# yirongjie/mllm

Measured on AMD Instinct MI355X. Metric: decode tok/s + prefill ms (448px img), Qwen2-VL-2B INT4, 1 GPU, higher is better.
Workload: dtype int8xint4->int32, fp32 accumulate (Q8_K x Q4_K); 1 GPU; demo_qwen2_vl Qwen2-VL-2B Q4_K: 448x448 image (1024 patches) + 24-token prompt prefill (S=282), then greedy decode, KV limit 800; parallelism=single, rccl_world=1, kv_segments=5

## Files before the change

mllm_amd/csrc/common.h:

```cpp
#pragma once
#include <hip/hip_runtime.h>
#include <hip/hip_fp16.h>
#include <stdint.h>

#include "../../include/mllm_hip.h"

namespace mllm_hip {

void set_error(const char *what, hipError_t e, const char *file, int line);
void set_error_msg(const char *fmt, ...);
int check_launch(const char *what, const char *file, int line);

#define MH_CHECK(expr)                                                        \
    do {                                                                      \
        hipError_t _e = (expr);                                               \
        if (_e != hipSuccess) {                                               \
            ::mllm_hip::set_error(#expr, _e, __FILE__, __LINE__);             \
            return MLLM_HIP_ERR_HIP;                                          \
        }                                                                     \
    } while (0)
#define MH_LAUNCH_OK(name) ::mllm_hip::check_launch(name, __FILE__, __LINE__)

static inline hipStream_t as_stream(void *s) { return reinterpret_cast<hipStream_t>(s); }

// ... 139 lines not shown
}
__device__ __forceinline__ float wave_scan_max(float v) {
    v = fmaxf(v, MH_DPPF(v, v, 0x111 , 0xF));
    v = fmaxf(v, MH_DPPF(v, v, 0x112 , 0xF));
    v = fmaxf(v, MH_DPPF(v, v, 0x114 , 0xF));
    v = fmaxf(v, MH_DPPF(v, v, 0x118 , 0xF));
    v = fmaxf(v, MH_DPPF(v, v, DPP_BCAST15, 0xA));
    v = fmaxf(v, MH_DPPF(v, v, DPP_BCAST31, 0xC));
    return v;
}
__device__ __forceinline__ float wave_shift_up(float v, float first) { return MH_DPPF(first, v, 0x138 , 0xF); }

__device__ __forceinline__ void unpack_q4k_scales(uint32_t u0, uint32_t u1, uint32_t u2, uint32_t sc8[2], uint32_t mn8[2]) {
    const uint32_t kmask1 = 0x3f3f3f3f, kmask2 = 0x0f0f0f0f, kmask3 = 0x03030303;
    mn8[1] = ((u2 >> 4) & kmask2) | (((u1 >> 6) & kmask3) << 4);
    mn8[0] = u1 & kmask1;
    sc8[1] = (u2 & kmask2) | (((u0 >> 6) & kmask3) << 4);
    sc8[0] = u0 & kmask1;
}
__device__ __forceinline__ int byte_of(const uint32_t v[2], int j) { return (v[j >> 2] >> (8 * (j & 3))) & 0xff; }

__device__ __forceinline__ int dot4(int a, int b, int c) { return __builtin_amdgcn_sdot4(a, b, c, false); }

constexpr size_t Q4KP_W_PER_BLK = 32 * 512, Q4KP_M_PER_BLK = 32 * 4 * 8, Q4KP_D_PER_BLK = 32 * 8;
__host__ __device__ static inline size_t q4kp_tile_blocks(int rows, int nb) { return (size_t)((rows + 31) / 32) * nb; }
static inline size_t q4kp_bytes(int rows, int K) {
    const size_t tb = q4kp_tile_blocks(rows, K / 256);
    return tb * (Q4KP_W_PER_BLK + Q4KP_M_PER_BLK + Q4KP_D_PER_BLK);
}
constexpr size_t Q4KW_Q_PER_BLK = 4096, Q4KW_S_PER_BLK = 512, Q4KW_M_PER_BLK = 1024, Q4KW_D_PER_BLK = 256;
static inline size_t q4kw_bytes(int rows, int K) { return q4kp_tile_blocks(rows, K / 256) * (Q4KW_Q_PER_BLK + Q4KW_S_PER_BLK + Q4KW_M_PER_BLK + Q4KW_D_PER_BLK); }

}

#include "ref_arith.h"
```

mllm_amd/csrc/kernels_elem.hip:

```cpp
#include <algorithm>
#include <vector>
#include <cmath>
#include <cstring>

#include "common.h"
#include "decode_launch.h"

namespace mllm_hip {

__device__ __forceinline__ void wave_quant_q8k(float4 v, int lane, int8_t *qs_blk, float *d_out, int16_t *bsums_blk) {
    unsigned abits;
    const float mx = q8k_first_max(v, abits);
    const float iscale = abits ? __fdiv_rn(-128.0f, mx) : 0.0f, dd = abits ? __fdiv_rn(1.0f, iscale) : 0.0f;
    uint32_t b[4];
    q8k_round4(v, iscale, b);
    const uint32_t packed = q8k_bytes(b);
    reinterpret_cast<uint32_t *>(qs_blk)[lane] = packed;
    const int s = group4_sum(q8k_sum4(packed));
    if ((lane & 3) == 0) bsums_blk[lane >> 2] = (int16_t)s;
    if (lane == 0) *d_out = dd;
}

typedef _Float16 v4h_t __attribute__((ext_vector_type(4)));
#ifndef QP_WAVES
#define QP_WAVES 8
#endif
__device__ __forceinline__ void wave_quant_pack(float4 v, int lane, bool live, uint8_t *pack, size_t tb, int nb, int m, int i) {
    unsigned abits;
    const float mx = q8k_first_max(v, abits);
    const bool nz = live && abits != 0;
    const float iscale = nz ? __fdiv_rn(-128.0f, mx) : 0.0f, dd = nz ? __fdiv_rn(1.0f, iscale) : 0.0f;
    uint32_t b[4];
    q8k_round4(v, iscale, b);
    f32x2_t q01, q23;
    q8k_floats(b, q01, q23);
    const size_t tile = (size_t)(m >> 5) * nb + i;
    const int mi = m & 31, j = lane >> 4, hf = (lane >> 3) & 1, t = lane & 7;
    v4h_t o;
    o[0] = (_Float16)q01.x; o[1] = (_Float16)q01.y; o[2] = (_Float16)q23.x; o[3] = (_Float16)q23.y;
    *reinterpret_cast<v4h_t *>(pack + ((((tile * 8 + t) * 2 + (j >> 1)) * 64 + (j & 1) * 32 + mi) * 16) + hf * 8) = o;
    const int s8 = group8_sum(q8k_sum4(q8k_bytes(b)));
    const int s8n = MH_DPP(0, s8, 0x108 , 0xF);
    if ((lane & 15) == 0) {
        v4h_t mo;
        mo[0] = (_Float16)(float)(s8 & ~1); mo[1] = (_Float16)(float)(s8 & 1);
        mo[2] = (_Float16)(float)(s8n & ~1); mo[3] = (_Float16)(float)(s8n & 1);
        *reinterpret_cast<v4h_t *>(pack + tb * Q4KP_W_PER_BLK + ((tile * 4 + (lane >> 4)) * 32 + mi) * 8) = mo;
    }
    if (lane == 0) *reinterpret_cast<float *>(pack + tb * (Q4KP_W_PER_BLK + Q4KP_M_PER_BLK) + (tile * 32 + mi) * 4) = dd;
}
__global__ __launch_bounds__(64 * QP_WAVES) void quantize_q8k_pack_kernel(const float *__restrict__ x, uint8_t *__restrict__ pack, int M, int nb) {
    const int lane = threadIdx.x & 63;
    const int64_t blk = (int64_t)blockIdx.x * QP_WAVES + (threadIdx.x >> 6);
    const int Mp = (M + 31) & ~31;
    if (blk >= (int64_t)Mp * nb) return;
    const int mi = (int)(blk & 31), i = (int)((blk >> 5) % nb), m = (int)((blk >> 5) / nb) * 32 + mi;
    const bool live = m < M;
    float4 v = make_float4(0, 0, 0, 0);
    if (live) v = reinterpret_cast<const float4 *>(x + ((int64_t)m * nb + i) * 256)[lane];
    wave_quant_pack(v, lane, live, pack, q4kp_tile_blocks(M, nb), nb, m, i);
}
__global__ __launch_bounds__(256) void quantize_q8k_kernel(const float *__restrict__ x, int8_t *__restrict__ qs, float *__restrict__ d,
                                                           int16_t *__restrict__ bsums, int64_t n_blocks) {
    const int lane = threadIdx.x & 63;
    const int64_t blk = (int64_t)blockIdx.x * 4 + (threadIdx.x >> 6);
    if (blk >= n_blocks) return;
    const float4 v = reinterpret_cast<const float4 *>(x + blk * 256)[lane];
    wave_quant_q8k(v, lane, qs + blk * 256, d + blk, bsums + blk * 16);
}

__global__ __launch_bounds__(256) void quantize_q80_kernel(const float *__restrict__ x, int8_t *__restrict__ qs, uint16_t *__restrict__ d, int64_t n_blocks) {
// ... 1292 lines not shown
```

mllm_amd/csrc/kernels_linear.hip:

```cpp
#include <type_traits>
#include <atomic>

#include "common.h"
#include "q4k_dot.h"
#include "q40_dot.h"

namespace mllm_hip {

typedef int v4i __attribute__((ext_vector_type(4)));
typedef int v16i __attribute__((ext_vector_type(16)));
typedef float v16f __attribute__((ext_vector_type(16)));

template <int NSTEPS, int ROWS>
__global__ __launch_bounds__(256) void gemv_q4k_kernel(const uint8_t *__restrict__ W, const float *__restrict__ bias, const int8_t *__restrict__ xqs,
                                                       const float *__restrict__ xd, const int16_t *__restrict__ xbsums, void *__restrict__ y, int y_f16,
                                                       const float *__restrict__ residual, int N, int nb, int rows_per_wave, int M, int64_t ldy) {
    __shared__ float2 tab_all[4 * (ROWS < 4 ? ROWS : 4) * NSTEPS * 8 * Q4K_SLOTS];
    const int lane = threadIdx.x & 63, g = lane >> 3, wid = threadIdx.x >> 6;
    const int wave = blockIdx.x * 4 + wid;
    float2 *tab = tab_all + wid * (ROWS < 4 ? ROWS : 4) * NSTEPS * 8 * Q4K_SLOTS;
    Q4KAct<NSTEPS> A;
    if (M == 1) q4k_load_act_planes<NSTEPS>(A, xqs, xd, xbsums, nb, lane);
    const int qoff = q4k_lane_qoff(lane);
    const int row0 = wave * rows_per_wave;
// ... 135 lines not shown
    float *Ad = reinterpret_cast<float *>(out + tb * (Q4KP_W_PER_BLK + Q4KP_M_PER_BLK));
    const size_t tile = (size_t)(m >> 5) * nb + i;
    const int min_ = m & 31, p = j >> 1, h = j & 1;
    const bool live = m < M;
    const int8_t *xb = xqs + ((int64_t)(live ? m : 0) * nb + i) * 256 + 64 * j;
    const uint4 la = *reinterpret_cast<const uint4 *>(xb), lb = *reinterpret_cast<const uint4 *>(xb + 16);
    const uint4 ha = *reinterpret_cast<const uint4 *>(xb + 32), hb = *reinterpret_cast<const uint4 *>(xb + 48);
    const uint32_t lo[8] = {la.x, la.y, la.z, la.w, lb.x, lb.y, lb.z, lb.w}, hi[8] = {ha.x, ha.y, ha.z, ha.w, hb.x, hb.y, hb.z, hb.w};
#pragma unroll
    for (int t = 0; t < 8; ++t) {
        v8h o;
#pragma unroll
        for (int bb = 0; bb < 4; ++bb) {
            o[bb] = (_Float16)(live ? (float)(int8_t)((lo[t] >> (8 * bb)) & 0xff) : 0.0f);
            o[4 + bb] = (_Float16)(live ? (float)(int8_t)((hi[t] >> (8 * bb)) & 0xff) : 0.0f);
        }
        Ax[((tile * 8 + t) * 2 + p) * 64 + h * 32 + min_] = o;
    }
    const int16_t *bs = xbsums + ((int64_t)(live ? m : 0) * nb + i) * 16 + 4 * j;
    const int q0 = live ? (int)bs[0] + (int)bs[1] : 0, q1 = live ? (int)bs[2] + (int)bs[3] : 0;
    v4h mo;
    mo[0] = (_Float16)(float)(q0 & ~1); mo[1] = (_Float16)(float)(q0 & 1);
    mo[2] = (_Float16)(float)(q1 & ~1); mo[3] = (_Float16)(float)(q1 & 1);
    Am[(tile * 4 + j) * 32 + min_] = mo;
    if (j == 0) Ad[tile * 32 + min_] = live ? xd[(int64_t)m * nb + i] : 0.0f;
}

constexpr int GQ_SLOT = 16384, GQ_SLOTS = 4, GQ_LDS = GQ_SLOT * GQ_SLOTS;
typedef _Float16 v2h __attribute__((ext_vector_type(2)));
__device__ __forceinline__ uint32_t and_or(uint32_t q, uint32_t mask_s, uint32_t magic_v) {
    uint32_t r;
    asm("v_and_or_b32 %0, %1, %2, %3" : "=v"(r) : "v"(q), "s"(mask_s), "v"(magic_v));
    return r;
}
__device__ __forceinline__ v8h q4_expand(uint32_t q, v2h s, v2h o1024, v2h o64, uint32_t m0f, uint32_t mf0, uint32_t k1024, uint32_t k64) {
    const uint32_t t = q >> 8;
    const v2h d0 = __builtin_bit_cast(v2h, and_or(q, m0f, k1024)), d1 = __builtin_bit_cast(v2h, and_or(q, mf0, k64));
    const v2h d2 = __builtin_bit_cast(v2h, and_or(t, m0f, k1024)), d3 = __builtin_bit_cast(v2h, and_or(t, mf0, k64));
    const v2h w0 = __builtin_elementwise_fma(d0, (v2h){s[0], s[0]}, (v2h){o1024[0], o1024[0]});
    const v2h w1 = __builtin_elementwise_fma(d1, (v2h){s[0], s[0]}, (v2h){o64[0], o64[0]});
    const v2h w2 = __builtin_elementwise_fma(d2, (v2h){s[1], s[1]}, (v2h){o1024[1], o1024[1]});
    const v2h w3 = __builtin_elementwise_fma(d3, (v2h){s[1], s[1]}, (v2h){o64[1], o64[1]});
    return (v8h){w0[0], w0[1], w1[0], w1[1], w2[0], w2[1], w3[0], w3[1]};
}
#if defined(MLLM_HIP_STAMPS)
constexpr int GQ_ST_HS = 12, GQ_ST_N = 8, GQ_ST_WG = 64;
__device__ unsigned long long g_gq_stamps[GQ_ST_WG * (4 * GQ_ST_HS * GQ_ST_N + 8)];
#define GQS(i) do { __builtin_amdgcn_sched_barrier(0); const unsigned long long t_ = __builtin_amdgcn_s_memtime(); if (lane == 0 && st_hs < GQ_ST_HS) st_lds[(wid * GQ_ST_HS + st_hs) * GQ_ST_N + (i)] = t_; __builtin_amdgcn_sched_barrier(0); } while (0)
#else
#define GQS(i) do { } while (0)
#endif
#if defined(GQ_NO_RETIRE)
constexpr int GQ_RET = 1;
#else
constexpr int GQ_RET = 16;
#endif
#if defined(GQ_NO_MFMA)
#define GQ_MFMA(a, b, c) (c)
#else
#define GQ_MFMA(a, b, c) __builtin_amdgcn_mfma_f32_32x32x16_f16(a, b, c, 0, 0, 0)
#endif
#if defined(GQ_NO_EXPAND)
#define GQ_EXPAND(q, s, o1, o2) __builtin_bit_cast(v8h, (u32x4){q, q, q, q})
#else
#define GQ_EXPAND(q, s, o1, o2) q4_expand(q, s, o1, o2, m0f, mf0, k1024, k64)
#endif
__global__ __launch_bounds__(256, 2) void gemm_q4k_kernel(const uint8_t *__restrict__ Wp, const uint8_t *__restrict__ Xp, const float *__restrict__ bias,
                                                          void *__restrict__ y, int y_f16, int64_t ldy, const float *__restrict__ residual, int M, int N,
                                                          int nb, int m_fastest) {
    extern __shared__ __attribute__((aligned(16))) char ring[];
    const int GXt = (N + 63) / 64, MTt = (M + 31) / 32;
    const int tile_x = m_fastest ? (int)blockIdx.x / MTt : (int)blockIdx.x % GXt, tile_y = m_fastest ? (int)blockIdx.x % MTt : (int)blockIdx.x / GXt;
    const int lane = threadIdx.x & 63, wid = __builtin_amdgcn_readfirstlane(threadIdx.x >> 6);
#if defined(MLLM_HIP_STAMPS)
    __shared__ unsigned long long st_lds[4 * GQ_ST_HS * GQ_ST_N];
    int st_hs = 0;
    unsigned long long st_rt[6];
    st_rt[0] = __builtin_amdgcn_s_memrealtime();
    st_rt[2] = 0;
    for (int i = threadIdx.x; i < 4 * GQ_ST_HS * GQ_ST_N; i += 256) st_lds[i] = 0;
#endif
#if defined(GQ_STAGGER)
    if ((((int)blockIdx.x >> 8) & 1) && (int)blockIdx.x < 512) {
#pragma unroll 1
        for (int i = 0; i < GQ_STAGGER; i += 100) __builtin_amdgcn_s_sleep(100);
    }
#endif
    const int col = lane & 31, h = lane >> 5;
    const int NT = (N + 31) / 32;
    const int nw = wid >> 1, ch = wid & 1;
    const int mt = tile_y, nt = tile_x * 2 + nw;
    const bool active = nt < NT;
    const size_t tbw = q4kp_tile_blocks(N, nb), tbx = q4kp_tile_blocks(M, nb);
    const int nts0 = min(tile_x * 2, NT - 1), nts1 = min(tile_x * 2 + 1, NT - 1);
    const uint8_t *XpM = Xp + tbx * Q4KP_W_PER_BLK, *XpD = XpM + tbx * Q4KP_M_PER_BLK;
    const uint8_t *WpS = Wp + tbw * Q4KW_Q_PER_BLK, *WpM = WpS + tbw * Q4KW_S_PER_BLK, *WpD = WpM + tbw * Q4KW_M_PER_BLK;
    const unsigned ring0 = (unsigned)(size_t)ring;
    auto uniform_ptr = [](const uint8_t *ptr) __attribute__((always_inline)) {
        const uint32_t plo = (uint32_t)__builtin_amdgcn_readfirstlane((int)(uint32_t)(uint64_t)ptr), phi = (uint32_t)__builtin_amdgcn_readfirstlane((int)(uint32_t)((uint64_t)ptr >> 32));
        return reinterpret_cast<const uint8_t *>(((uint64_t)phi << 32) | (uint64_t)plo);
    };
    const uint8_t *sa0 = uniform_ptr(Xp + (size_t)mt * nb * Q4KP_W_PER_BLK + (size_t)wid * 1024);
    const uint8_t *sa1 = uniform_ptr(Xp + (size_t)mt * nb * Q4KP_W_PER_BLK + (size_t)(4 + wid) * 1024);
    const uint8_t *sq = uniform_ptr(Wp + (size_t)(nw ? nts1 : nts0) * nb * Q4KW_Q_PER_BLK + (size_t)ch * 1024);
    const uint8_t *pe = Xp + lane * 16, *po = Xp + lane * 16;
    unsigned se = 0, so = 0;
    if (wid == 0) {
        pe = lane < 8    ? XpD + (size_t)mt * nb * 128 + lane * 16
             : lane < 24 ? WpD + (size_t)nts0 * nb * 256 + (lane - 8) * 16
             : lane < 40 ? WpD + (size_t)nts1 * nb * 256 + (lane - 24) * 16
                         : Xp + lane * 16;
        se = lane < 8 ? 128u : (lane < 40 ? 256u : 0u);
        po = XpM + (size_t)mt * nb * 1024 + lane * 16;
        so = 1024u;
    } else if (wid == 1) {
        pe = WpS + (size_t)(lane < 32 ? nts0 : nts1) * nb * 512 + (lane & 31) * 16;
        se = 512u;
        po = WpM + (size_t)nts0 * nb * 1024 + lane * 16;
        so = 1024u;
    } else if (wid == 2) {
        po = WpM + (size_t)nts1 * nb * 1024 + lane * 16;
        so = 1024u;
    }
    unsigned voffA = (unsigned)lane * 16u, voffB = (unsigned)lane * 16u;
    unsigned islot = ring0;
    auto issue = [&](int hb) __attribute__((always_inline)) {
        const unsigned d0 = __builtin_amdgcn_readfirstlane(islot + (unsigned)wid * 1024u);
        const uint8_t *pa = hb == 0 ? pe : po;
        unsigned keep;
        asm volatile("s_mov_b32 %0, m0\n\ts_mov_b32 m0, %3\n\ts_nop 0\n\tglobal_load_lds_dwordx4 %1, %4\n\t"
                     "s_add_u32 m0, m0, 0x1000\n\ts_nop 0\n\tglobal_load_lds_dwordx4 %1, %5\n\t"
                     "s_add_u32 m0, m0, 0x1000\n\ts_nop 0\n\tglobal_load_lds_dwordx4 %2, %6\n\t"
                     "s_add_u32 m0, m0, 0x1000\n\ts_nop 0\n\tglobal_load_lds_dwordx4 %7, off\n\ts_mov_b32 m0, %0"
                     : "=&s"(keep) : "v"(voffA), "v"(voffB), "s"(d0), "s"(sa0), "s"(sa1), "s"(sq), "v"(pa) : "memory", "scc");
        voffA += 8192u;
        voffB += 2048u;
        islot = islot + (unsigned)GQ_SLOT == ring0 + (unsigned)GQ_LDS ? ring0 : islot + (unsigned)GQ_SLOT;
        if (hb == 0) pe += se; else po += so;
    };
    const int TS = 2 * nb;
    issue(0);
    issue(1);
    if (TS > 2) issue(0);
    __builtin_amdgcn_sched_barrier(0);
#if defined(MLLM_HIP_STAMPS)
    st_rt[1] = __builtin_amdgcn_s_memrealtime();
#endif
    v16f acc[4], accm[2];
#pragma unroll
    for (int t = 0; t < 4; ++t)
#pragma unroll
        for (int r = 0; r < 16; ++r) acc[t][r] = 0.0f;
#pragma unroll
    for (int u = 0; u < 2; ++u)
#pragma unroll
        for (int r = 0; r < 16; ++r) accm[u][r] = 0.0f;
    v16f zero;
#pragma unroll
    for (int r = 0; r < 16; ++r) zero[r] = 0.0f;
    typedef float f32x4 __attribute__((ext_vector_type(4)));
    typedef float f32x2 __attribute__((ext_vector_type(2)));
    typedef unsigned u32x2 __attribute__((ext_vector_type(2)));
    typedef unsigned u32x4 __attribute__((ext_vector_type(4)));
    float dd[16], dm[16];
#pragma unroll
    for (int r = 0; r < 16; ++r) dd[r] = dm[r] = 0.0f;
    v16f cp0 = zero, cp1 = zero;
    v2h sc[2] = {{0, 0}, {0, 0}}, o1024[2] = {{0, 0}, {0, 0}}, o64[2] = {{0, 0}, {0, 0}};
    const uint32_t k1024 = 0x64006400u, k64 = 0x54005400u;
    const uint32_t m0f = __builtin_amdgcn_readfirstlane(0x000F000F), mf0 = __builtin_amdgcn_readfirstlane(0x00F000F0);
    const unsigned lA = ring0 + (unsigned)(ch * 4096 + lane * 16), lQ = ring0 + (unsigned)((8 + 2 * nw + ch) * 1024 + lane * 16);
    const unsigned lX = ring0 + (unsigned)(12288 + 16 * h), lW = ring0 + (unsigned)(12288 + 128 + nw * 256 + col * 8), lS = ring0 + (unsigned)(13312 + nw * 512 + lane * 8);
    const unsigned lAm = ring0 + (unsigned)(12288 + col * 8 + 2 * ch * 256), lBm = ring0 + (unsigned)(13312 + nw * 1024 + col * 8 + 2 * ch * 256);
    unsigned cslot = 0;
    auto step = [&](auto HB, auto REM) __attribute__((always_inline)) {
        constexpr int hb = decltype(HB)::value, rem = decltype(REM)::value;
        GQS(0);
        if (rem >= 2) asm volatile("s_waitcnt vmcnt(8)" ::: "memory");
        else if (rem == 1) asm volatile("s_waitcnt vmcnt(4)" ::: "memory");
        else asm volatile("s_waitcnt vmcnt(0)" ::: "memory");
        GQS(1);
#if !defined(GQ_NO_BAR)
        __builtin_amdgcn_s_barrier();
#endif
        asm volatile("" ::: "memory");
        GQS(2);
#if defined(MLLM_HIP_STAMPS)
        if (st_rt[2] == 0) st_rt[2] = __builtin_amdgcn_s_memrealtime();
#endif
#if !defined(GQ_NO_DMA)
        if (rem >= 3) issue(1 - hb);
#endif
        GQS(3);
        if (active) {
            typedef __attribute__((address_space(3))) const char *lds_cp;
            const unsigned cs = __builtin_amdgcn_readfirstlane(cslot);
            const u32x4 qv = *reinterpret_cast<__attribute__((address_space(3))) const u32x4 *>((lds_cp)(size_t)(lQ + cs));
            u32x2 sraw;
            if (hb == 0) sraw = *reinterpret_cast<__attribute__((address_space(3))) const u32x2 *>((lds_cp)(size_t)(lS + cs));
            const __attribute__((address_space(3))) v8h *A = reinterpret_cast<__attribute__((address_space(3))) const v8h *>((lds_cp)(size_t)(lA + cs));
            const v8h a0 = A[0], a2 = A[128], a1 = A[64], a3 = A[192];
            f32x2 dwv;
            f32x4 dx[4];
            v4h a4[2], b4[2];
            if (hb == 0) {
                dwv = *reinterpret_cast<__attribute__((address_space(3))) const f32x2 *>((lds_cp)(size_t)(lW + cs));
#pragma unroll
                for (int g4 = 0; g4 < 4; ++g4) dx[g4] = *reinterpret_cast<__attribute__((address_space(3))) const f32x4 *>((lds_cp)(size_t)(lX + cs) + 32 * g4);
            } else {
                const __attribute__((address_space(3))) v4h *Am = reinterpret_cast<__attribute__((address_space(3))) const v4h *>((lds_cp)(size_t)(lAm + cs));
                const __attribute__((address_space(3))) v4h *Bm = reinterpret_cast<__attribute__((address_space(3))) const v4h *>((lds_cp)(size_t)(lBm + cs));
#pragma unroll
                for (int k = 0; k < 2; ++k) { a4[k] = Am[k * 32]; b4[k] = Bm[k * 32]; }
            }
            GQS(4);
#pragma unroll
            for (int r = 0; r < GQ_RET; ++r) acc[2 * (1 - hb)][r] = __fmaf_rn(dd[r], cp0[r], acc[2 * (1 - hb)][r]);
            if (hb == 0) {
                const v2h n1024 = {(_Float16)-1024.0f, (_Float16)-1024.0f}, n64 = {(_Float16)-64.0f, (_Float16)-64.0f};
#pragma unroll
                for (int p = 0; p < 2; ++p) {
                    const unsigned sv = p == 0 ? sraw.x : sraw.y;
                    sc[p] = __builtin_bit_cast(v2h, sv);
                    o1024[p] = sc[p] * n1024;
                    o64[p] = sc[p] * n64;
                }
            }
            v16f cm0, cm1;
            if (hb == 1) {
                v8h am[2], bm[2];
#pragma unroll
                for (int k = 0; k < 2; ++k) {
                    const u32x2 ua = __builtin_bit_cast(u32x2, a4[k]), ub = __builtin_bit_cast(u32x2, b4[k]);
                    const u32x4 wa = {h == 0 ? ua[0] : 0u, h == 0 ? ua[1] : 0u, 0u, 0u}, wb = {h == 0 ? ub[0] : 0u, h == 0 ? ub[1] : 0u, 0u, 0u};
                    am[k] = __builtin_bit_cast(v8h, wa); bm[k] = __builtin_bit_cast(v8h, wb);
                }
                cm0 = GQ_MFMA(am[0], bm[0], zero);
                cm1 = GQ_MFMA(am[1], bm[1], zero);
            }
            const v8h b0 = GQ_EXPAND(qv[0], sc[0], o1024[0], o64[0]);
            cp0 = GQ_MFMA(a0, b0, zero);
#pragma unroll
            for (int r = 0; r < GQ_RET; ++r) acc[2 * (1 - hb) + 1][r] = __fmaf_rn(dd[r], cp1[r], acc[2 * (1 - hb) + 1][r]);
            const v8h b2 = GQ_EXPAND(qv[2], sc[0], o1024[0], o64[0]);
            cp1 = GQ_MFMA(a2, b2, zero);
            const v8h b1 = GQ_EXPAND(qv[1], sc[1], o1024[1], o64[1]);
            cp0 = GQ_MFMA(a1, b1, cp0);
            const v8h b3 = GQ_EXPAND(qv[3], sc[1], o1024[1], o64[1]);
            cp1 = GQ_MFMA(a3, b3, cp1);
            if (hb == 0) {
#pragma unroll
                for (int g4 = 0; g4 < 4; ++g4)
#pragma unroll
                    for (int e = 0; e < 4; ++e) {
                        dd[4 * g4 + e] = dx[g4][e] * dwv[0];
                        dm[4 * g4 + e] = (-dx[g4][e]) * dwv[1];
                    }
            } else {
#pragma unroll
                for (int r = 0; r < 16; ++r) {
                    accm[0][r] = __fmaf_rn(dm[r], cm0[r], accm[0][r]);
                    accm[1][r] = __fmaf_rn(dm[r], cm1[r], accm[1][r]);
                }
            }
        }
        GQS(6);
#if defined(MLLM_HIP_STAMPS)
        ++st_hs;
#endif
        cslot = cslot + (unsigned)GQ_SLOT == (unsigned)GQ_LDS ? 0u : cslot + (unsigned)GQ_SLOT;
    };
    using std::integral_constant;
#pragma unroll 1
    for (int i = 0; i + 2 < nb; ++i) {
        step(integral_constant<int, 0>{}, integral_constant<int, 3>{});
        step(integral_constant<int, 1>{}, integral_constant<int, 3>{});
    }
    if (nb >= 2) {
        step(integral_constant<int, 0>{}, integral_constant<int, 3>{});
        step(integral_constant<int, 1>{}, integral_constant<int, 2>{});
    }
    step(integral_constant<int, 0>{}, integral_constant<int, 1>{});
    step(integral_constant<int, 1>{}, integral_constant<int, 0>{});
    if (active) {
#pragma unroll
        for (int r = 0; r < 16; ++r) {
            acc[2][r] = __fmaf_rn(dd[r], cp0[r], acc[2][r]);
            acc[3][r] = __fmaf_rn(dd[r], cp1[r], acc[3][r]);
        }
    }
#if defined(MLLM_HIP_STAMPS)
    st_rt[3] = __builtin_amdgcn_s_memrealtime();
#endif
    float x[16], yv[16];
#pragma unroll
    for (int r = 0; r < 16; ++r) { x[r] = acc[0][r] + acc[2][r]; yv[r] = acc[1][r] + acc[3][r]; }
    __syncthreads();
    float *xch = reinterpret_cast<float *>(ring) + (size_t)nw * 64 * 64 + lane;
    const int n = nt * 32 + col;
    auto finish = [&](auto R0) __attribute__((always_inline)) {
        constexpr int r0 = decltype(R0)::value, p0 = 8 - r0;
#pragma unroll
        for (int j = 0; j < 8; ++j) {
            const int r = p0 + j;
            xch[r * 64] = x[r]; xch[(16 + r) * 64] = yv[r]; xch[(32 + r) * 64] = accm[0][r]; xch[(48 + r) * 64] = accm[1][r];
        }
        __syncthreads();
#if defined(MLLM_HIP_STAMPS)
        st_rt[4] = __builtin_amdgcn_s_memrealtime();
#endif
        if (!active || n >= N) return;
        float v[8];
#pragma unroll
        for (int j = 0; j < 8; ++j) {
            const int r = r0 + j;
            const float hs = (x[r] + xch[r * 64]) + (yv[r] + xch[(16 + r) * 64]);
            v[j] = hs + ((accm[0][r] + xch[(32 + r) * 64]) + (accm[1][r] + xch[(48 + r) * 64]));
        }
        if (bias) {
            const float bv = bias[n];
#pragma unroll
            for (int j = 0; j < 8; ++j) v[j] = v[j] + bv;
        }
        const int mb = mt * 32 + 4 * h;
        if (y_f16) {
            uint16_t *yp = reinterpret_cast<uint16_t *>(y) + n;
#pragma unroll
            for (int j = 0; j < 8; ++j) {
                const int m = mb + ((r0 + j) & 3) + 8 * ((r0 + j) >> 2);
                if (m < M) yp[(int64_t)m * ldy] = f2h(v[j]);
            }
        } else {
            float *yp = reinterpret_cast<float *>(y) + n;
            if (residual) {
                float res[8];
#pragma unroll
                for (int j = 0; j < 8; ++j) res[j] = residual[(int64_t)min(mb + ((r0 + j) & 3) + 8 * ((r0 + j) >> 2), M - 1) * ldy + n];
#pragma unroll
                for (int j = 0; j < 8; ++j) v[j] = v[j] + res[j];
            }
#pragma unroll
            for (int j = 0; j < 8; ++j) {
                const int m = mb + ((r0 + j) & 3) + 8 * ((r0 + j) >> 2);
                if (m < M) yp[(int64_t)m * ldy] = v[j];
            }
        }
    };
    if (ch == 0) finish(std::integral_constant<int, 0>{}); else finish(std::integral_constant<int, 8>{});
#if defined(MLLM_HIP_STAMPS)
    {
        const int wg = blockIdx.x;
        if (wg % 37 == 0 && wg / 37 < GQ_ST_WG) {
            unsigned long long *dst = g_gq_stamps + (size_t)(wg / 37) * (4 * GQ_ST_HS * GQ_ST_N + 8);
            for (int i = threadIdx.x; i < 4 * GQ_ST_HS * GQ_ST_N; i += 256) dst[i] = st_lds[i];
            asm volatile("s_waitcnt vmcnt(0)" ::: "memory");
            st_rt[5] = __builtin_amdgcn_s_memrealtime();
            if (threadIdx.x == 0) {
                unsigned long long *tail = dst + 4 * GQ_ST_HS * GQ_ST_N;
                for (int i = 0; i < 6; ++i) tail[i] = st_rt[i];
                tail[6] = __builtin_amdgcn_s_getreg(63492); tail[7] = __builtin_amdgcn_s_getreg(63508);
            }
        }
    }
#endif
}

#if defined(MLLM_HIP_STAMPS)
extern "C" int mllm_hip_debug_read_gemm_stamps(unsigned long long *host, int n) {
    return hipMemcpyFromSymbol(host, HIP_SYMBOL(g_gq_stamps), (size_t)n * 8) == hipSuccess ? 0 : -1;
}
#endif

constexpr int F32_TM = 8, F32_TN = 4;
#define SWZ_XOR(v, k) __int_as_float(__builtin_amdgcn_ds_swizzle(__float_as_int(v), 0x1f | ((k) << 10)))
__global__ __launch_bounds__(256) void gemm_f32_kernel(const float *__restrict__ W, const float *__restrict__ bias, const float *__restrict__ x,
                                                       float *__restrict__ y, int64_t ldy, int M, int N, int K) {
    const int c = threadIdx.x & 31, gi = threadIdx.x >> 5;
    const int m0 = blockIdx.y * (2 * F32_TM) + (gi >> 2) * F32_TM, n0 = blockIdx.x * (4 * F32_TN) + (gi & 3) * F32_TN;
    const float *xr[F32_TM], *wr[F32_TN];
#pragma unroll
    for (int i = 0; i < F32_TM; ++i) xr[i] = x + (int64_t)min(m0 + i, M - 1) * K;
#pragma unroll
    for (int j = 0; j < F32_TN; ++j) wr[j] = W + (int64_t)min(n0 + j, N - 1) * K;
    float acc[F32_TM][F32_TN];
#pragma unroll
    for (int i = 0; i < F32_TM; ++i)
#pragma unroll
        for (int j = 0; j < F32_TN; ++j) acc[i][j] = 0.0f;
    const int np = K & ~31;
    for (int k = c; k < np; k += 32) {
        float xv[F32_TM], wv[F32_TN];
#pragma unroll
        for (int i = 0; i < F32_TM; ++i) xv[i] = xr[i][k];
#pragma unroll
// ... 391 lines not shown
```

Measured before the change: 1206 tok/s.

## Restructure Q4_K GEMM LDS ring layout and DMA addressing to cut loop bookkeeping

Reworks the prefill Q4_K MFMA GEMM's LDS staging. The per-step ring-slot modulo arithmetic is replaced by ping-pong base pointers that flip each super-block. DMA issues now use immediate offsets instead of m0 increments, and the activation min-sum plane is widened to 64 entries (zero-padded), so wave 3 also gets a DMA stream. Debug stamp and ablation macros are removed and a script is added to count loop instructions. The aim is fewer scalar and vector bookkeeping instructions per super-block, at the cost of a larger packed activation buffer and extra zero writes.

Measured after the change: 1205 tok/s. No clear change (-0.0%).

```diff
diff --git a/mllm_amd/csrc/common.h b/mllm_amd/csrc/common.h
--- a/mllm_amd/csrc/common.h
+++ b/mllm_amd/csrc/common.h
@@ -185,7 +185,7 @@
 
 __device__ __forceinline__ int dot4(int a, int b, int c) { return __builtin_amdgcn_sdot4(a, b, c, false); }
 
-constexpr size_t Q4KP_W_PER_BLK = 32 * 512, Q4KP_M_PER_BLK = 32 * 4 * 8, Q4KP_D_PER_BLK = 32 * 8;
+constexpr size_t Q4KP_W_PER_BLK = 32 * 512, Q4KP_M_PER_BLK = 64 * 4 * 8, Q4KP_D_PER_BLK = 32 * 8;
 __host__ __device__ static inline size_t q4kp_tile_blocks(int rows, int nb) { return (size_t)((rows + 31) / 32) * nb; }
 static inline size_t q4kp_bytes(int rows, int K) {
     const size_t tb = q4kp_tile_blocks(rows, K / 256);
diff --git a/mllm_amd/csrc/kernels_elem.hip b/mllm_amd/csrc/kernels_elem.hip
--- a/mllm_amd/csrc/kernels_elem.hip
+++ b/mllm_amd/csrc/kernels_elem.hip
@@ -45,8 +45,10 @@
         v4h_t mo;
         mo[0] = (_Float16)(float)(s8 & ~1); mo[1] = (_Float16)(float)(s8 & 1);
         mo[2] = (_Float16)(float)(s8n & ~1); mo[3] = (_Float16)(float)(s8n & 1);
-        *reinterpret_cast<v4h_t *>(pack + tb * Q4KP_W_PER_BLK + ((tile * 4 + (lane >> 4)) * 32 + mi) * 8) = mo;
-    }
+        *reinterpret_cast<v4h_t *>(pack + tb * Q4KP_W_PER_BLK + ((tile * 4 + (lane >> 4)) * 64 + mi) * 8) = mo;
+    }
+    if ((lane & 15) == 8)
+        *reinterpret_cast<v4h_t *>(pack + tb * Q4KP_W_PER_BLK + ((tile * 4 + (lane >> 4)) * 64 + 32 + mi) * 8) = (v4h_t){(_Float16)0.0f, (_Float16)0.0f, (_Float16)0.0f, (_Float16)0.0f};
     if (lane == 0) *reinterpret_cast<float *>(pack + tb * (Q4KP_W_PER_BLK + Q4KP_M_PER_BLK) + (tile * 32 + mi) * 4) = dd;
 }
 __global__ __launch_bounds__(64 * QP_WAVES) void quantize_q8k_pack_kernel(const float *__restrict__ x, uint8_t *__restrict__ pack, int M, int nb) {
diff --git a/mllm_amd/csrc/kernels_linear.hip b/mllm_amd/csrc/kernels_linear.hip
--- a/mllm_amd/csrc/kernels_linear.hip
+++ b/mllm_amd/csrc/kernels_linear.hip
@@ -181,7 +181,8 @@
     v4h mo;
     mo[0] = (_Float16)(float)(q0 & ~1); mo[1] = (_Float16)(float)(q0 & 1);
     mo[2] = (_Float16)(float)(q1 & ~1); mo[3] = (_Float16)(float)(q1 & 1);
-    Am[(tile * 4 + j) * 32 + min_] = mo;
+    Am[(tile * 4 + j) * 64 + min_] = mo;
+    Am[(tile * 4 + j) * 64 + 32 + min_] = (v4h){(_Float16)0.0f, (_Float16)0.0f, (_Float16)0.0f, (_Float16)0.0f};
     if (j == 0) Ad[tile * 32 + min_] = live ? xd[(int64_t)m * nb + i] : 0.0f;
 }
 
@@ -202,28 +203,6 @@
     const v2h w3 = __builtin_elementwise_fma(d3, (v2h){s[1], s[1]}, (v2h){o64[1], o64[1]});
     return (v8h){w0[0], w0[1], w1[0], w1[1], w2[0], w2[1], w3[0], w3[1]};
 }
-#if defined(MLLM_HIP_STAMPS)
-constexpr int GQ_ST_HS = 12, GQ_ST_N = 8, GQ_ST_WG = 64;
-__device__ unsigned long long g_gq_stamps[GQ_ST_WG * (4 * GQ_ST_HS * GQ_ST_N + 8)];
-#define GQS(i) do { __builtin_amdgcn_sched_barrier(0); const unsigned long long t_ = __builtin_amdgcn_s_memtime(); if (lane == 0 && st_hs < GQ_ST_HS) st_lds[(wid * GQ_ST_HS + st_hs) * GQ_ST_N + (i)] = t_; __builtin_amdgcn_sched_barrier(0); } while (0)
-#else
-#define GQS(i) do { } while (0)
-#endif
-#if defined(GQ_NO_RETIRE)
-constexpr int GQ_RET = 1;
-#else
-constexpr int GQ_RET = 16;
-#endif
-#if defined(GQ_NO_MFMA)
-#define GQ_MFMA(a, b, c) (c)
-#else
-#define GQ_MFMA(a, b, c) __builtin_amdgcn_mfma_f32_32x32x16_f16(a, b, c, 0, 0, 0)
-#endif
-#if defined(GQ_NO_EXPAND)
-#define GQ_EXPAND(q, s, o1, o2) __builtin_bit_cast(v8h, (u32x4){q, q, q, q})
-#else
-#define GQ_EXPAND(q, s, o1, o2) q4_expand(q, s, o1, o2, m0f, mf0, k1024, k64)
-#endif
 __global__ __launch_bounds__(256, 2) void gemm_q4k_kernel(const uint8_t *__restrict__ Wp, const uint8_t *__restrict__ Xp, const float *__restrict__ bias,
                                                           void *__restrict__ y, int y_f16, int64_t ldy, const float *__restrict__ residual, int M, int N,
                                                           int nb, int m_fastest) {
@@ -231,20 +210,6 @@
     const int GXt = (N + 63) / 64, MTt = (M + 31) / 32;
     const int tile_x = m_fastest ? (int)blockIdx.x / MTt : (int)blockIdx.x % GXt, tile_y = m_fastest ? (int)blockIdx.x % MTt : (int)blockIdx.x / GXt;
     const int lane = threadIdx.x & 63, wid = __builtin_amdgcn_readfirstlane(threadIdx.x >> 6);
-#if defined(MLLM_HIP_STAMPS)
-    __shared__ unsigned long long st_lds[4 * GQ_ST_HS * GQ_ST_N];
-    int st_hs = 0;
-    unsigned long long st_rt[6];
-    st_rt[0] = __builtin_amdgcn_s_memrealtime();
-    st_rt[2] = 0;
-    for (int i = threadIdx.x; i < 4 * GQ_ST_HS * GQ_ST_N; i += 256) st_lds[i] = 0;
-#endif
-#if defined(GQ_STAGGER)
-    if ((((int)blockIdx.x >> 8) & 1) && (int)blockIdx.x < 512) {
-#pragma unroll 1
-        for (int i = 0; i < GQ_STAGGER; i += 100) __builtin_amdgcn_s_sleep(100);
-    }
-#endif
     const int col = lane & 31, h = lane >> 5;
     const int NT = (N + 31) / 32;
     const int nw = wid >> 1, ch = wid & 1;
@@ -255,56 +220,64 @@
     const uint8_t *XpM = Xp + tbx * Q4KP_W_PER_BLK, *XpD = XpM + tbx * Q4KP_M_PER_BLK;
     const uint8_t *WpS = Wp + tbw * Q4KW_Q_PER_BLK, *WpM = WpS + tbw * Q4KW_S_PER_BLK, *WpD = WpM + tbw * Q4KW_M_PER_BLK;
     const unsigned ring0 = (unsigned)(size_t)ring;
-    auto uniform_ptr = [](const uint8_t *ptr) __attribute__((always_inline)) {
-        const uint32_t plo = (uint32_t)__builtin_amdgcn_readfirstlane((int)(uint32_t)(uint64_t)ptr), phi = (uint32_t)__builtin_amdgcn_readfirstlane((int)(uint32_t)((uint64_t)ptr >> 32));
+    auto uniform_ptr = [](uintptr_t ptr) __attribute__((always_inline)) {
+        const uint32_t plo = (uint32_t)__builtin_amdgcn_readfirstlane((int)(uint32_t)ptr), phi = (uint32_t)__builtin_amdgcn_readfirstlane((int)(uint32_t)((uint64_t)ptr >> 32));
         return reinterpret_cast<const uint8_t *>(((uint64_t)phi << 32) | (uint64_t)plo);
     };
-    const uint8_t *sa0 = uniform_ptr(Xp + (size_t)mt * nb * Q4KP_W_PER_BLK + (size_t)wid * 1024);
-    const uint8_t *sa1 = uniform_ptr(Xp + (size_t)mt * nb * Q4KP_W_PER_BLK + (size_t)(4 + wid) * 1024);
-    const uint8_t *sq = uniform_ptr(Wp + (size_t)(nw ? nts1 : nts0) * nb * Q4KW_Q_PER_BLK + (size_t)ch * 1024);
-    const uint8_t *pe = Xp + lane * 16, *po = Xp + lane * 16;
+    const uint8_t *sa0 = uniform_ptr((uintptr_t)Xp + (size_t)mt * nb * Q4KP_W_PER_BLK + (size_t)wid * 1024);
+    const uint8_t *sa1 = uniform_ptr((uintptr_t)Xp + (size_t)mt * nb * Q4KP_W_PER_BLK + (size_t)(4 + wid) * 1024 - 1024);
+    const uint8_t *sq = uniform_ptr((uintptr_t)Wp + (size_t)(nw ? nts1 : nts0) * nb * Q4KW_Q_PER_BLK + (size_t)ch * 1024 - 2048);
+    uintptr_t pe = (uintptr_t)Xp + lane * 16, po = (uintptr_t)Xp + lane * 16;
     unsigned se = 0, so = 0;
     if (wid == 0) {
-        pe = lane < 8    ? XpD + (size_t)mt * nb * 128 + lane * 16
-             : lane < 24 ? WpD + (size_t)nts0 * nb * 256 + (lane - 8) * 16
-             : lane < 40 ? WpD + (size_t)nts1 * nb * 256 + (lane - 24) * 16
-                         : Xp + lane * 16;
+        pe = (uintptr_t)(lane < 8    ? XpD + (size_t)mt * nb * 128 + lane * 16
+                         : lane < 24 ? WpD + (size_t)nts0 * nb * 256 + (lane - 8) * 16
+                         : lane < 40 ? WpD + (size_t)nts1 * nb * 256 + (lane - 24) * 16
+                                     : Xp + lane * 16);
         se = lane < 8 ? 128u : (lane < 40 ? 256u : 0u);
-        po = XpM + (size_t)mt * nb * 1024 + lane * 16;
-        so = 1024u;
+        po = (uintptr_t)(XpM + (size_t)mt * nb * Q4KP_M_PER_BLK + lane * 16);
+        so = (unsigned)Q4KP_M_PER_BLK;
     } else if (wid == 1) {
-        pe = WpS + (size_t)(lane < 32 ? nts0 : nts1) * nb * 512 + (lane & 31) * 16;
+        pe = (uintptr_t)(WpS + (size_t)(lane < 32 ? nts0 : nts1) * nb * 512 + (lane & 31) * 16);
         se = 512u;
-        po = WpM + (size_t)nts0 * nb * 1024 + lane * 16;
+        po = (uintptr_t)(WpM + (size_t)nts0 * nb * 1024 + lane * 16);
         so = 1024u;
     } else if (wid == 2) {
-        po = WpM + (size_t)nts1 * nb * 1024 + lane * 16;
+        po = (uintptr_t)(WpM + (size_t)nts1 * nb * 1024 + lane * 16);
         so = 1024u;
-    }
+    } else {
+        po = (uintptr_t)(XpM + (size_t)mt * nb * Q4KP_M_PER_BLK + 1024 + lane * 16);
+        so = (unsigned)Q4KP_M_PER_BLK;
+    }
+    pe -= 3072;
+    po -= 3072;
     unsigned voffA = (unsigned)lane * 16u, voffB = (unsigned)lane * 16u;
-    unsigned islot = ring0;
-    auto issue = [&](int hb) __attribute__((always_inline)) {
-        const unsigned d0 = __builtin_amdgcn_readfirstlane(islot + (unsigned)wid * 1024u);
-        const uint8_t *pa = hb == 0 ? pe : po;
+    const unsigned dbase = __builtin_amdgcn_readfirstlane(ring0 + (unsigned)wid * 4096u);
+    auto issue = [&](auto HB, unsigned d0) __attribute__((always_inline)) {
+        constexpr int hb = decltype(HB)::value;
+        const uintptr_t pa = hb == 0 ? pe : po;
         unsigned keep;
-        asm volatile("s_mov_b32 %0, m0\n\ts_mov_b32 m0, %3\n\ts_nop 0\n\tglobal_load_lds_dwordx4 %1, %4\n\t"
-                     "s_add_u32 m0, m0, 0x1000\n\ts_nop 0\n\tglobal_load_lds_dwordx4 %1, %5\n\t"
-                     "s_add_u32 m0, m0, 0x1000\n\ts_nop 0\n\tglobal_load_lds_dwordx4 %2, %6\n\t"
-                     "s_add_u32 m0, m0, 0x1000\n\ts_nop 0\n\tglobal_load_lds_dwordx4 %7, off\n\ts_mov_b32 m0, %0"
-                     : "=&s"(keep) : "v"(voffA), "v"(voffB), "s"(d0), "s"(sa0), "s"(sa1), "s"(sq), "v"(pa) : "memory", "scc");
+        asm volatile("s_mov_b32 %0, m0\n\ts_mov_b32 m0, %3\n\ts_nop 0\n\t"
+                     "global_load_lds_dwordx4 %1, %4\n\t"
+                     "global_load_lds_dwordx4 %1, %5 offset:1024\n\t"
+                     "global_load_lds_dwordx4 %2, %6 offset:2048\n\t"
+                     "global_load_lds_dwordx4 %7, off offset:3072\n\ts_mov_b32 m0, %0"
+                     : "=&s"(keep) : "v"(voffA), "v"(voffB), "s"(d0), "s"(sa0), "s"(sa1), "s"(sq), "v"(pa) : "memory");
         voffA += 8192u;
         voffB += 2048u;
-        islot = islot + (unsigned)GQ_SLOT == ring0 + (unsigned)GQ_LDS ? ring0 : islot + (unsigned)GQ_SLOT;
         if (hb == 0) pe += se; else po += so;
     };
+    using std::integral_constant;
+    typedef integral_constant<int, 0> I0;
+    typedef integral_constant<int, 1> I1;
+    typedef integral_constant<int, 2> I2;
+    typedef integral_constant<int, 3> I3;
+    unsigned dA = dbase + 3u * GQ_SLOT, dB = dbase, sdl = 2u * GQ_SLOT;
     const int TS = 2 * nb;
-    issue(0);
-    issue(1);
-    if (TS > 2) issue(0);
+    issue(I0{}, dbase);
+    issue(I1{}, dbase + (unsigned)GQ_SLOT);
+    if (TS > 2) issue(I0{}, dbase + 2u * GQ_SLOT);
     __builtin_amdgcn_sched_barrier(0);
-#if defined(MLLM_HIP_STAMPS)
-    st_rt[1] = __builtin_amdgcn_s_memrealtime();
-#endif
     v16f acc[4], accm[2];
 #pragma unroll
     for (int t = 0; t < 4; ++t)
@@ -328,129 +301,109 @@
     v2h sc[2] = {{0, 0}, {0, 0}}, o1024[2] = {{0, 0}, {0, 0}}, o64[2] = {{0, 0}, {0, 0}};
     const uint32_t k1024 = 0x64006400u, k64 = 0x54005400u;
     const uint32_t m0f = __builtin_amdgcn_readfirstlane(0x000F000F), mf0 = __builtin_amdgcn_readfirstlane(0x00F000F0);
-    const unsigned lA = ring0 + (unsigned)(ch * 4096 + lane * 16), lQ = ring0 + (unsigned)((8 + 2 * nw + ch) * 1024 + lane * 16);
-    const unsigned lX = ring0 + (unsigned)(12288 + 16 * h), lW = ring0 + (unsigned)(12288 + 128 + nw * 256 + col * 8), lS = ring0 + (unsigned)(13312 + nw * 512 + lane * 8);
-    const unsigned lAm = ring0 + (unsigned)(12288 + col * 8 + 2 * ch * 256), lBm = ring0 + (unsigned)(13312 + nw * 1024 + col * 8 + 2 * ch * 256);
-    unsigned cslot = 0;
+    typedef __attribute__((address_space(3))) const char *lds_cp;
+    unsigned lA = ring0 + (unsigned)(ch * 1024 + lane * 16), lQ = ring0 + (unsigned)((4 * wid + 2) * 1024 + lane * 16);
+    unsigned lX = ring0 + (unsigned)(3072 + 16 * h), lW = ring0 + (unsigned)(3072 + 128 + nw * 256 + col * 8), lS = ring0 + (unsigned)(7168 + nw * 512 + lane * 8);
+    unsigned lAm = ring0 + (unsigned)((ch ? 15360 : 3072) + lane * 8), lBm = ring0 + (unsigned)(7168 + nw * 4096 + col * 8 + ch * 512);
     auto step = [&](auto HB, auto REM) __attribute__((always_inline)) {
-        constexpr int hb = decltype(HB)::value, rem = decltype(REM)::value;
-        GQS(0);
+        constexpr int hb = decltype(HB)::value, rem = decltype(REM)::value, so_ = hb * GQ_SLOT;
+        const lds_cp pA = (lds_cp)(size_t)lA, pQ = (lds_cp)(size_t)lQ, pX = (lds_cp)(size_t)lX, pW = (lds_cp)(size_t)lW, pS = (lds_cp)(size_t)lS;
+        const lds_cp pAm = (lds_cp)(size_t)lAm, pBm = (lds_cp)(size_t)lBm;
         if (rem >= 2) asm volatile("s_waitcnt vmcnt(8)" ::: "memory");
         else if (rem == 1) asm volatile("s_waitcnt vmcnt(4)" ::: "memory");
         else asm volatile("s_waitcnt vmcnt(0)" ::: "memory");
-        GQS(1);
-#if !defined(GQ_NO_BAR)
         __builtin_amdgcn_s_barrier();
-#endif
         asm volatile("" ::: "memory");
-        GQS(2);
-#if defined(MLLM_HIP_STAMPS)
-        if (st_rt[2] == 0) st_rt[2] = __builtin_amdgcn_s_memrealtime();
-#endif
-#if !defined(GQ_NO_DMA)
-        if (rem >= 3) issue(1 - hb);
-#endif
-        GQS(3);
-        if (active) {
-            typedef __attribute__((address_space(3))) const char *lds_cp;
-            const unsigned cs = __builtin_amdgcn_readfirstlane(cslot);
-            const u32x4 qv = *reinterpret_cast<__attribute__((address_space(3))) const u32x4 *>((lds_cp)(size_t)(lQ + cs));
-            u32x2 sraw;
-            if (hb == 0) sraw = *reinterpret_cast<__attribute__((address_space(3))) const u32x2 *>((lds_cp)(size_t)(lS + cs));
-            const __attribute__((address_space(3))) v8h *A = reinterpret_cast<__attribute__((address_space(3))) const v8h *>((lds_cp)(size_t)(lA + cs));
-            const v8h a0 = A[0], a2 = A[128], a1 = A[64], a3 = A[192];
-            f32x2 dwv;
-            f32x4 dx[4];
-            v4h a4[2], b4[2];
-            if (hb == 0) {
-                dwv = *reinterpret_cast<__attribute__((address_space(3))) const f32x2 *>((lds_cp)(size_t)(lW + cs));
-#pragma unroll
-                for (int g4 = 0; g4 < 4; ++g4) dx[g4] = *reinterpret_cast<__attribute__((address_space(3))) const f32x4 *>((lds_cp)(size_t)(lX + cs) + 32 * g4);
-            } else {
-                const __attribute__((address_space(3))) v4h *Am = reinterpret_cast<__attribute__((address_space(3))) const v4h *>((lds_cp)(size_t)(lAm + cs));
-                const __attribute__((address_space(3))) v4h *Bm = reinterpret_cast<__attribute__((address_space(3))) const v4h *>((lds_cp)(size_t)(lBm + cs));
-#pragma unroll
-                for (int k = 0; k < 2; ++k) { a4[k] = Am[k * 32]; b4[k] = Bm[k * 32]; }
-            }
-            GQS(4);
-#pragma unroll
-            for (int r = 0; r < GQ_RET; ++r) acc[2 * (1 - hb)][r] = __fmaf_rn(dd[r], cp0[r], acc[2 * (1 - hb)][r]);
-            if (hb == 0) {
-                const v2h n1024 = {(_Float16)-1024.0f, (_Float16)-1024.0f}, n64 = {(_Float16)-64.0f, (_Float16)-64.0f};
-#pragma unroll
-                for (int p = 0; p < 2; ++p) {
-                    const unsigned sv = p == 0 ? sraw.x : sraw.y;
-                    sc[p] = __builtin_bit_cast(v2h, sv);
-                    o1024[p] = sc[p] * n1024;
-                    o64[p] = sc[p] * n64;
+        if (rem >= 3) issue(integral_constant<int, 1 - hb>{}, hb == 0 ? dA : dB);
+        __builtin_amdgcn_sched_barrier(0);
+        const u32x4 qv = *reinterpret_cast<__attribute__((address_space(3))) const u32x4 *>(pQ + so_);
+        u32x2 sraw;
+        if (hb == 0) sraw = *reinterpret_cast<__attribute__((address_space(3))) const u32x2 *>(pS + so_);
+        const __attribute__((address_space(3))) v8h *A = reinterpret_cast<__attribute__((address_space(3))) const v8h *>(pA + so_);
+        const v8h a0 = A[0], a2 = A[512], a1 = A[256], a3 = A[768];
+        f32x2 dwv;
+        f32x4 dx[4];
+        v4h a4[2], b4[2];
+        if (hb == 0) {
+            dwv = *reinterpret_cast<__attribute__((address_space(3))) const f32x2 *>(pW + so_);
+#pragma unroll
+            for (int g4 = 0; g4 < 4; ++g4) dx[g4] = *reinterpret_cast<__attribute__((address_space(3))) const f32x4 *>(pX + so_ + 32 * g4);
+        } else {
+            const volatile __attribute__((address_space(3))) v4h *Am = reinterpret_cast<const volatile __attribute__((address_space(3))) v4h *>(pAm + so_);
+            const volatile __attribute__((address_space(3))) v4h *Bm = reinterpret_cast<const volatile __attribute__((address_space(3))) v4h *>(pBm + so_);
+#pragma unroll
+            for (int k = 0; k < 2; ++k) { a4[k] = Am[k * 64]; b4[k] = Bm[k * 32]; }
+        }
+#pragma unroll
+        for (int r = 0; r < 16; ++r) acc[2 * (1 - hb)][r] = __fmaf_rn(dd[r], cp0[r], acc[2 * (1 - hb)][r]);
+        if (hb == 0) {
+            const v2h n1024 = {(_Float16)-1024.0f, (_Float16)-1024.0f}, n64 = {(_Float16)-64.0f, (_Float16)-64.0f};
+#pragma unroll
+            for (int p = 0; p < 2; ++p) {
+                const unsigned sv = p == 0 ? sraw.x : sraw.y;
+                sc[p] = __builtin_bit_cast(v2h, sv);
+                o1024[p] = sc[p] * n1024;
+                o64[p] = sc[p] * n64;
+            }
+        }
+        v16f cm0, cm1;
+        if (hb == 1) {
+            v8h am[2], bm[2];
+#pragma unroll
+            for (int k = 0; k < 2; ++k) {
+                const u32x2 ua = __builtin_bit_cast(u32x2, a4[k]), ub = __builtin_bit_cast(u32x2, b4[k]);
+                const u32x4 wa = {ua[0], ua[1], 0u, 0u}, wb = {ub[0], ub[1], 0u, 0u};
+                am[k] = __builtin_bit_cast(v8h, wa); bm[k] = __builtin_bit_cast(v8h, wb);
+            }
+            cm0 = __builtin_amdgcn_mfma_f32_32x32x16_f16(am[0], bm[0], zero, 0, 0, 0);
+            cm1 = __builtin_amdgcn_mfma_f32_32x32x16_f16(am[1], bm[1], zero, 0, 0, 0);
+        }
+        const v8h b0 = q4_expand(qv[0], sc[0], o1024[0], o64[0], m0f, mf0, k1024, k64);
+        cp0 = __builtin_amdgcn_mfma_f32_32x32x16_f16(a0, b0, zero, 0, 0, 0);
+#pragma unroll
+        for (int r = 0; r < 16; ++r) acc[2 * (1 - hb) + 1][r] = __fmaf_rn(dd[r], cp1[r], acc[2 * (1 - hb) + 1][r]);
+        const v8h b2 = q4_expand(qv[2], sc[0], o1024[0], o64[0], m0f, mf0, k1024, k64);
+        cp1 = __builtin_amdgcn_mfma_f32_32x32x16_f16(a2, b2, zero, 0, 0, 0);
+        const v8h b1 = q4_expand(qv[1], sc[1], o1024[1], o64[1], m0f, mf0, k1024, k64);
+        cp0 = __builtin_amdgcn_mfma_f32_32x32x16_f16(a1, b1, cp0, 0, 0, 0);
+        const v8h b3 = q4_expand(qv[3], sc[1], o1024[1], o64[1], m0f, mf0, k1024, k64);
+        cp1 = __builtin_amdgcn_mfma_f32_32x32x16_f16(a3, b3, cp1, 0, 0, 0);
+        if (hb == 0) {
+#pragma unroll
+            for (int g4 = 0; g4 < 4; ++g4)
+#pragma unroll
+                for (int e = 0; e < 4; ++e) {
+                    dd[4 * g4 + e] = dx[g4][e] * dwv[0];
+                    dm[4 * g4 + e] = (-dx[g4][e]) * dwv[1];
                 }
-            }
-            v16f cm0, cm1;
-            if (hb == 1) {
-                v8h am[2], bm[2];
-#pragma unroll
-                for (int k = 0; k < 2; ++k) {
-                    const u32x2 ua = __builtin_bit_cast(u32x2, a4[k]), ub = __builtin_bit_cast(u32x2, b4[k]);
-                    const u32x4 wa = {h == 0 ? ua[0] : 0u, h == 0 ? ua[1] : 0u, 0u, 0u}, wb = {h == 0 ? ub[0] : 0u, h == 0 ? ub[1] : 0u, 0u, 0u};
-                    am[k] = __builtin_bit_cast(v8h, wa); bm[k] = __builtin_bit_cast(v8h, wb);
-                }
-                cm0 = GQ_MFMA(am[0], bm[0], zero);
-                cm1 = GQ_MFMA(am[1], bm[1], zero);
-            }
-            const v8h b0 = GQ_EXPAND(qv[0], sc[0], o1024[0], o64[0]);
-            cp0 = GQ_MFMA(a0, b0, zero);
-#pragma unroll
-            for (int r = 0; r < GQ_RET; ++r) acc[2 * (1 - hb) + 1][r] = __fmaf_rn(dd[r], cp1[r], acc[2 * (1 - hb) + 1][r]);
-            const v8h b2 = GQ_EXPAND(qv[2], sc[0], o1024[0], o64[0]);
-            cp1 = GQ_MFMA(a2, b2, zero);
-            const v8h b1 = GQ_EXPAND(qv[1], sc[1], o1024[1], o64[1]);
-            cp0 = GQ_MFMA(a1, b1, cp0);
-            const v8h b3 = GQ_EXPAND(qv[3], sc[1], o1024[1], o64[1]);
-            cp1 = GQ_MFMA(a3, b3, cp1);
-            if (hb == 0) {
-#pragma unroll
-                for (int g4 = 0; g4 < 4; ++g4)
-#pragma unroll
-                    for (int e = 0; e < 4; ++e) {
-                        dd[4 * g4 + e] = dx[g4][e] * dwv[0];
-                        dm[4 * g4 + e] = (-dx[g4][e]) * dwv[1];
-                    }
-            } else {
-#pragma unroll
-                for (int r = 0; r < 16; ++r) {
-                    accm[0][r] = __fmaf_rn(dm[r], cm0[r], accm[0][r]);
-                    accm[1][r] = __fmaf_rn(dm[r], cm1[r], accm[1][r]);
-                }
-            }
-        }
-        GQS(6);
-#if defined(MLLM_HIP_STAMPS)
-        ++st_hs;
-#endif
-        cslot = cslot + (unsigned)GQ_SLOT == (unsigned)GQ_LDS ? 0u : cslot + (unsigned)GQ_SLOT;
+        } else {
+#pragma unroll
+            for (int r = 0; r < 16; ++r) {
+                accm[0][r] = __fmaf_rn(dm[r], cm0[r], accm[0][r]);
+                accm[1][r] = __fmaf_rn(dm[r], cm1[r], accm[1][r]);
+            }
+            if (rem > 0) {
+                lA += sdl; lQ += sdl; lX += sdl; lW += sdl; lS += sdl; lAm += sdl; lBm += sdl;
+                dA -= sdl; dB += sdl; sdl = 0u - sdl;
+            }
+        }
     };
-    using std::integral_constant;
 #pragma unroll 1
     for (int i = 0; i + 2 < nb; ++i) {
-        step(integral_constant<int, 0>{}, integral_constant<int, 3>{});
-        step(integral_constant<int, 1>{}, integral_constant<int, 3>{});
+        step(I0{}, I3{});
+        step(I1{}, I3{});
     }
     if (nb >= 2) {
-        step(integral_constant<int, 0>{}, integral_constant<int, 3>{});
-        step(integral_constant<int, 1>{}, integral_constant<int, 2>{});
-    }
-    step(integral_constant<int, 0>{}, integral_constant<int, 1>{});
-    step(integral_constant<int, 1>{}, integral_constant<int, 0>{});
-    if (active) {
-#pragma unroll
-        for (int r = 0; r < 16; ++r) {
-            acc[2][r] = __fmaf_rn(dd[r], cp0[r], acc[2][r]);
-            acc[3][r] = __fmaf_rn(dd[r], cp1[r], acc[3][r]);
-        }
-    }
-#if defined(MLLM_HIP_STAMPS)
-    st_rt[3] = __builtin_amdgcn_s_memrealtime();
-#endif
+        step(I0{}, I3{});
+        step(I1{}, I2{});
+    }
+    step(I0{}, I1{});
+    step(I1{}, I0{});
+#pragma unroll
+    for (int r = 0; r < 16; ++r) {
+        acc[2][r] = __fmaf_rn(dd[r], cp0[r], acc[2][r]);
+        acc[3][r] = __fmaf_rn(dd[r], cp1[r], acc[3][r]);
+    }
     float x[16], yv[16];
 #pragma unroll
     for (int r = 0; r < 16; ++r) { x[r] = acc[0][r] + acc[2][r]; yv[r] = acc[1][r] + acc[3][r]; }
@@ -465,9 +418,6 @@
             xch[r * 64] = x[r]; xch[(16 + r) * 64] = yv[r]; xch[(32 + r) * 64] = accm[0][r]; xch[(48 + r) * 64] = accm[1][r];
         }
         __syncthreads();
-#if defined(MLLM_HIP_STAMPS)
-        st_rt[4] = __builtin_amdgcn_s_memrealtime();
-#endif
         if (!active || n >= N) return;
         float v[8];
 #pragma unroll
@@ -506,29 +456,7 @@
         }
     };
     if (ch == 0) finish(std::integral_constant<int, 0>{}); else finish(std::integral_constant<int, 8>{});
-#if defined(MLLM_HIP_STAMPS)
-    {
-        const int wg = blockIdx.x;
-        if (wg % 37 == 0 && wg / 37 < GQ_ST_WG) {
-            unsigned long long *dst = g_gq_stamps + (size_t)(wg / 37) * (4 * GQ_ST_HS * GQ_ST_N + 8);
-            for (int i = threadIdx.x; i < 4 * GQ_ST_HS * GQ_ST_N; i += 256) dst[i] = st_lds[i];
-            asm volatile("s_waitcnt vmcnt(0)" ::: "memory");
-            st_rt[5] = __builtin_amdgcn_s_memrealtime();
-            if (threadIdx.x == 0) {
-                unsigned long long *tail = dst + 4 * GQ_ST_HS * GQ_ST_N;
-                for (int i = 0; i < 6; ++i) tail[i] = st_rt[i];
-                tail[6] = __builtin_amdgcn_s_getreg(63492); tail[7] = __builtin_amdgcn_s_getreg(63508);
-            }
-        }
-    }
-#endif
-}
-
-#if defined(MLLM_HIP_STAMPS)
-extern "C" int mllm_hip_debug_read_gemm_stamps(unsigned long long *host, int n) {
-    return hipMemcpyFromSymbol(host, HIP_SYMBOL(g_gq_stamps), (size_t)n * 8) == hipSuccess ? 0 : -1;
-}
-#endif
+}
 
 constexpr int F32_TM = 8, F32_TN = 4;
 #define SWZ_XOR(v, k) __int_as_float(__builtin_amdgcn_ds_swizzle(__float_as_int(v), 0x1f | ((k) << 10)))
diff --git a/profiles/gemm_loop_count.py b/profiles/gemm_loop_count.py
--- /dev/null
+++ b/profiles/gemm_loop_count.py
@@ -0,0 +1,76 @@
+#!/usr/bin/env python3
+import collections
+import os
+import re
+import subprocess
+import sys
+import tempfile
+
+HERE = os.path.dirname(os.path.abspath(__file__))
+ARITH = ("v_and_or_b32", "v_pk_fma_f16", "v_lshrrev_b32", "v_pk_mul_f16", "v_pk_fma_f32", "v_fma_f32", "v_pk_mul_f32", "v_mul_f32")
+
+
+def classify(m: str) -> str:
+    if m.startswith("v_mfma"):
+        return "MFMA"
+    if m.startswith("global_load_lds"):
+        return "LDS-DMA"
+    if m.startswith("ds_read"):
+        return "LDS reads"
+    if m in ARITH or m[:-4] in ARITH:
+        return "VALU arithmetic"
+    if m.startswith("v_"):
+        return "VALU bookkeeping"
+    if m.startswith("s_"):
+        return "SALU"
+    return "other"
+
+
+def main() -> int:
+    src = sys.argv[1] if len(sys.argv) > 1 else os.path.join(HERE, "..", "mllm_amd", "csrc", "kernels_linear.hip")
+    hipcc = os.environ.get("HIPCC", "/opt/rocm/bin/hipcc")
+    with tempfile.TemporaryDirectory() as td:
+        out = os.path.join(td, "k.s")
+        subprocess.check_call([hipcc, "--offload-arch=gfx950", "-O3", "-std=c++17", "-ffp-contract=off", "--cuda-device-only", "-S", src, "-o", out])
+        text = open(out).read().splitlines()
+    start = next(i for i, l in enumerate(text) if re.match(r"_ZN8mllm_hip15gemm_q4k_kernel\w*:", l))
+    end = next(i for i in range(start, len(text)) if text[i].startswith(".Lfunc_end"))
+    body = text[start:end]
+    meta = {}
+    for l in text[end:]:
+        m = re.match(r"\s*;\s*(NumVgprs|NumAgprs|ScratchSize|Occupancy|NumSgprs|LDSByteSize):\s*(\d+)", l)
+        if m and m.group(1) not in meta:
+            meta[m.group(1)] = int(m.group(2))
+        if len(meta) == 6 or l.startswith("_ZN"):
+            break
+    labels = {m.group(1): i for i, l in enumerate(body) if (m := re.match(r"(\.LBB\d+_\d+):", l))}
+    insns = [(i, l.split()[0]) for i, l in enumerate(body) if l.startswith("\t") and not l.lstrip().startswith((".", ";")) and l.strip()]
+    best = None
+    for i, l in enumerate(body):
+        m = re.match(r"\ts_cbranch_\w+\s+(\.LBB\d+_\d+)", l) or re.match(r"\ts_branch\s+(\.LBB\d+_\d+)", l)
+        if not m or labels.get(m.group(1), len(body)) >= i:
+            continue
+        span = [mn for k, mn in insns if labels[m.group(1)] < k <= i]
+        nm, nd = sum(mn.startswith("v_mfma") for mn in span), sum(mn.startswith("global_load_lds") for mn in span)
+        if nd and (best is None or nm > best[0] or (nm == best[0] and len(span) < len(best[1]))):
+            best = (nm, span)
+    if best is None:
+        print("no loop with LDS-DMAs found")
+        return 1
+    nm, span = best
+    k = nm / 10.0
+    print(f"kernel: {meta}")
+    print(f"steady-state loop: {len(span)} instructions per trip, {nm} MFMAs = {k:g} super-block(s) per trip -> {len(span) / k:.1f} per super-block\n")
+    by = collections.defaultdict(collections.Counter)
+    for mn in span:
+        by[classify(mn)][re.sub(r"_e(32|64)$", "", mn)] += 1
+    print("| class | per trip | per super-block | of which (per trip) |\n|---|---|---|---|")
+    for c in ("MFMA", "LDS-DMA", "LDS reads", "VALU arithmetic", "VALU bookkeeping", "SALU", "other"):
+        if by[c]:
+            n = sum(by[c].values())
+            print(f"| {c} | {n} | {n / k:.1f} | " + ", ".join(f"`{mn}` {v}" for mn, v in by[c].most_common()) + " |")
+    return 0
+
+
+if __name__ == "__main__":
+    sys.exit(main())
```
